# ChristophReich1996/Multi-StyleGAN

Measured on AMD Instinct MI355X. Metric: training images/sec (G+D step, 256^2, seq=3x2ch), higher is better.
Workload: dtype bf16

## Files before the change

### include/msg_hip.h

```cpp
#ifndef MSG_HIP_H
#define MSG_HIP_H

#ifdef __cplusplus
extern "C" {
#endif

enum { MSG_OK = 0, MSG_EINVAL = -1, MSG_EUNSUPPORTED = -2, MSG_ELAUNCH = -3 };
enum { MSG_F32 = 0, MSG_BF16 = 1, MSG_F16 = 2, MSG_F64 = 3, MSG_F32_SPLIT = 4 };

#define MSG_ABI_VERSION 5
int msg_abi_version(void);
const char* msg_build_arch(void);
const char* msg_strerror(int code);

int msg_upfirdn2d(const void* x, const float* fir, void* y, int dtype,
                  int major, int in_h, int in_w, int minor, int kh, int kw,
                  int up_x, int up_y, int down_x, int down_y,
                  int pad_x0, int pad_x1, int pad_y0, int pad_y1, void* stream);

int msg_upfirdn2d_pitched(const void* x, const float* fir, void* y, int dtype,
                          int major, int in_h, int in_w, int minor, int in_pitch, int kh, int kw,
                          int up_x, int up_y, int down_x, int down_y,
                          int pad_x0, int pad_x1, int pad_y0, int pad_y1, void* stream);

int msg_upfirdn2d_pitched2(const void* x, const float* fir, void* y, int dtype,
                           int major, int in_h, int in_w, int minor, int in_pitch, int out_pitch, int kh, int kw,
                           int up_x, int up_y, int down_x, int down_y,
                           int pad_x0, int pad_x1, int pad_y0, int pad_y1, void* stream);

int msg_upfirdn2d_separable(const void* x, const float* fir_y, const float* fir_x, void* y, int dtype,
                            int major, int in_h, int in_w, int minor, int kh, int kw,
                            int pad_x0, int pad_x1, int pad_y0, int pad_y1, void* stream);

int msg_upfirdn2d_separable_act(const void* x, const float* fir_y, const float* fir_x, void* y, int dtype,
                                int major, int in_h, int in_w, int minor, int kh, int kw,
                                int pad_x0, int pad_x1, int pad_y0, int pad_y1,
                                const float* act_bias, const float* noise, const float* noise_weight,
                                int noise_batch, float alpha, float scale, void* stream);
int msg_upfirdn2d_separable_act_mask(const void* x, const float* fir_y, const float* fir_x, void* y, int dtype,
                                     int major, int in_h, int in_w, int minor, int kh, int kw,
                                     int pad_x0, int pad_x1, int pad_y0, int pad_y1,
                                     const float* act_bias, const float* noise, const float* noise_weight,
                                     int noise_batch, float alpha, float scale, unsigned char* mask, void* stream);

int msg_fused_bias_act(const void* x, const float* bias, const void* ref, void* y, int dtype,
                       long long size_x, int step_b, int size_b,
                       const float* noise, const float* noise_weight, int noise_batch, int pix,
                       int act, int grad, float alpha, float scale, void* stream);

long long msg_bias_act_backward_workspace(long long size_x, int step_b, int size_b, int has_noise);
int msg_bias_act_backward(const void* gy, const void* out, void* gx, int dtype,
                          long long size_x, int step_b, int size_b,
                          float* grad_bias, const float* noise, float* grad_noise_weight,
                          int noise_batch, int pix, float alpha, float scale,
                          float* ws, long long ws_floats, void* stream);
int msg_channel_sums(const void* x, float* sums, int dtype, long long size_x, int C, float* ws, long long ws_floats,
                     void* stream);
int msg_bias_act_backward_mask(const void* gy, const unsigned char* mask, int tile_m, int tile_n, void* gx, int dtype,
                               long long size_x, int size_b,
                               float* grad_bias, const float* noise, float* grad_noise_weight,
                               int noise_batch, int pix, float alpha, float scale,
                               float* ws, long long ws_floats, void* stream);
int msg_sum_rows(const float* part, float* out, long long rows, int cols, void* stream);
int msg_bias_act_backward_mask_head(const void* gy, const void* ghead, const float* whead, const float* style,
                                    float wscale, int n_head, const unsigned char* mask, int tile_m, int tile_n,
                                    void* gx, int dtype, long long size_x, int size_b,
                                    float* grad_bias, const float* noise, float* grad_noise_weight,
                                    int noise_batch, int pix, float alpha, float scale,
                                    float* ws, long long ws_floats, void* stream);

int msg_conv2d_fprop(const void* x, const void* w, const float* bias, void* y, int dtype,
                     int B, int IH, int IW, int Cx, int Ck, int OH, int OW, int N, int ldy,
                     int kh, int kw, int stride, int pad, int in_up, int pixel_shuffle,
                     long long w_batch_stride, void* stream);
int msg_conv2d_wgrad(const void* gy, const void* x, float* gw, int dtype,
                     int B, int IH, int IW, int Cx, int I, int OH, int OW, int ldgy, int O, int ldgw,
                     int kh, int kw, int stride, int pad, int pixel_shuffle,
                     int per_sample, int k_chunks, int oi_major, float gain,
                     float* ws, long long ws_floats, void* stream);
long long msg_conv2d_wgrad_workspace(int dtype, int B, int IH, int IW, int Cx, int I, int OH, int OW, int ldgy,
                                     int O, int ldgw, int kh, int kw, int stride, int pad, int pixel_shuffle,
                                     int per_sample, int k_chunks);

int msg_demod_coeff(const float* W, const float* s, float* d, int B, int O, int I, int taps,
                    float scale, float eps, void* stream);
int msg_scale_rows_cols(const float* base, const float* rowscale, const float* colscale, void* out,
                        int dtype, int B, int R, int T, int C, int Ck, float gain, void* stream);
int msg_modulate_weights(const float* base, const float* wsq, const float* style, void* out, float* d_out,
                         int dtype, int B, int R, int O, int T, int C, int Ck, float scale, float eps, void* stream);
int msg_modulate_backward(const float* gwk, const float* W, const float* s, const float* d, float* gW,
                          float* gs_part, int B, int O, int I, int taps, int ldg, int o_group,
                          float scale, void* stream);
int msg_scale_rows_cols2(const float* base, const float* row1, const float* col1, const float* row2, const float* col2,
                         void* out, int dtype, int B, int R, int T, int C, int Ck, float gain, void* stream);
int msg_modulate_backward2(const float* gwk, const float* W, const float* s, const float* d, const float* v,
                           float* gW, float* gs_part, int B, int O, int I, int taps, int ldg, int o_group,
                           float scale, void* stream);

int msg_relayout_weight(const float* w, void* fwd, void* dgrad, float* wsq, int dtype,
                        int O, int I, int T, int Ck, int Ok, int flip, int t_major, float gain, void* stream);

int msg_gather_taps(const void* x, void* y, int dtype, int B, int H, int W, int Cx, int C, int kh, int kw,
                    int pad, int Ko, void* stream);
int msg_fold_taps(const void* g, const void* add, void* gx, int dtype, int B, int H, int W, int Ko, int C, int kh, int kw,
                  int pad, int ldx, int ld_add, void* stream);

int msg_scaled_add(const void* a, const void* b, void* y, int dtype, long long n, float beta, float gain, void* stream);
int msg_rgb_skip_merge(const void* conv, int dtype, int ld, const float* bias, const float* skip, const float* fir,
                       float* out, int B, int C, int H, int W, void* stream);
int msg_rgb_skip_merge_backward(const float* g, void* g_conv, int dtype, int ld, float* g_skip, const float* fir,
                                int B, int C, int H, int W, void* stream);
int msg_gamma_merge(const void* a, const void* b, const float* gamma, void* y, int dtype, long long n, float gain, void* stream);
long long msg_gamma_merge_backward_workspace(void);
int msg_gamma_merge_backward(const void* gy, const void* a, const float* gamma, void* ga, void* gb, float* g_gamma, int dtype,
                             long long n, float gain, float* ws, void* stream);
int msg_scaled_add_rows(const void* a, const void* b, void* y, int dtype, long long rows, int cols,
                        long long lda, long long ldb, long long ldy, float beta, float gain, void* stream);

int msg_softmax_rows(const void* x, void* y, int dtype, long long rows, int cols, void* stream);
int msg_softmax_rows_backward(const void* y, const void* gy, void* gx, int dtype, long long rows, int cols,
                              void* stream);
int msg_softmax_rows_backward2(const void* y, const void* gy, const void* v, void* d_y, void* d_gy, int dtype,
                               long long rows, int cols, void* stream);

int msg_nonlocal_attention_supported(int B, int Nq, int Nk, int dk, int dv);
int msg_nonlocal_attention_fwd(const void* q, const void* k, const void* vt, void* o, float* lse, int dtype,
                               int B, int Nq, int Nk, int dk, int dv, void* stream);
int msg_maxpool2x2_fwd(const void* x, void* y, unsigned short* idx, int dtype, int B, int H, int W, int C, long long ldx,
                       void* stream);
int msg_maxpool2x2_bwd(const void* gy, const unsigned short* idx, void* gx, int dtype, int B, int H, int W, int C,
                       void* stream);
int msg_maxpool2x2_gather(const void* v, const unsigned short* idx, void* out, int dtype, int B, int H, int W, int C,
                          long long ldv, void* stream);

int msg_nonlocal_attention_bwd_splits(int B, int Nq, int Nk);
int msg_nonlocal_attention_bwd(const void* q, const void* qt, const void* k, const void* kt, const void* v,
                               const void* dO, const void* dOt, const void* o, const float* lse, float* delta,
                               void* dq, void* dk_out, void* dv_out, float* workspace, int dtype,
                               int B, int Nq, int Nk, int dk, int dv, void* stream);

int msg_affine_warp(const float* x, float* y, const float* angle_deg, float angle_const, const float* scale_xy,
                    const float* select_u, const float* p, int rot_prob, float cx, float cy, int padding,
                    int align_corners, int B, int C, int H, int W, int backward, void* workspace, void* stream);

long long msg_minibatch_stddev_workspace(int C, int H, int W, int groups, int dtype);
int msg_minibatch_stddev(const void* x, void* y, float* stat, float* workspace, int dtype,
                         int B, int C, int H, int W, int ldx, int ldy, int groups, float alpha, void* stream);
int msg_minibatch_stddev_backward(const void* x, const void* gy, const float* gstat, void* gx, int dtype,
                                  int B, int C, int H, int W, int ldx, int ldgy, int ldgx, int groups,
                                  float alpha, void* stream);

int msg_conv2d_fprop_act(const void* x, const void* w, void* y, int dtype,
                         int B, int IH, int IW, int Cx, int Ck, int OH, int OW, int N, int ldy,
                         int kh, int kw, int stride, int pad, long long w_batch_stride,
                         const float* act_bias, const float* noise, const float* noise_weight,
                         int noise_batch, float alpha, float scale, void* stream);
int msg_conv2d_fprop_act_mask(const void* x, const void* w, void* y, int dtype,
                              int B, int IH, int IW, int Cx, int Ck, int OH, int OW, int N, int ldy,
                              int kh, int kw, int stride, int pad, long long w_batch_stride,
                              const float* act_bias, const float* noise, const float* noise_weight,
                              int noise_batch, float alpha, float scale, unsigned char* mask, void* stream);

int msg_conv2d_fprop_residual(const void* x, const void* w, void* y, int dtype,
                              int B, int IH, int IW, int Cx, int Ck, int OH, int OW, int N, int ldy,
                              int kh, int kw, int stride, int pad, long long w_batch_stride,
                              const void* residual, int res_ld, float gain, void* stream);

long long msg_conv2d_fprop_act_backward_workspace(int dtype, int B, int IH, int IW, int Cx, int Ck, int OH, int OW,
                                                  int N, int kh, int kw, long long w_batch_stride, int has_noise);
int msg_conv2d_fprop_act_backward(const void* x, const void* w, void* y, int dtype,
                                  int B, int IH, int IW, int Cx, int Ck, int OH, int OW, int N, int ldy,
                                  int kh, int kw, int stride, int pad, long long w_batch_stride,
                                  const void* residual, int res_ld,
                                  const unsigned char* sign_mask, int mask_tile_m, int mask_tile_n,
                                  const void* sign_map, int sign_ld, float alpha, float scale,
// ... 50 lines not shown
```

### multi_stylegan_amd/conv_ops.py

```python
import math
import os
from typing import Optional, Tuple

import torch
from torch.autograd import Function

from . import _lib
from ._autograd import _derive


def _vec(dtype) -> int:
    return 8 if dtype == torch.bfloat16 else 4


def _round_up(n: int, m: int) -> int:
    return (n + m - 1) // m * m


def _padded_nhwc(b, c, h, w, dtype, device):
    cx = _round_up(c, _vec(dtype))
    buf = torch.empty((b, h, w, cx), dtype=dtype, device=device)
    if cx != c:
        buf[..., c:].zero_()
    return buf.permute(0, 3, 1, 2)[:, :c]
# ... 1498 lines not shown


class _ModConvGrad(Function):

    @staticmethod
    def forward(ctx, gy, x, weight, style, d, demodulate, upsample, g, scale, need):
        gx, gw, gs, gwk = _modconv_backward(x, weight, style, d, gy, demodulate, upsample, g, scale, need, keep_gwk=True)
        ctx.set_materialize_grads(False)
        ctx.save_for_backward(gy, x, weight, style, d, gwk)
        ctx.cfg = (demodulate, upsample, g, scale)
        return gx, gw, gs

    @staticmethod
    @torch.autograd.function.once_differentiable
    def backward(ctx, a, cot_w, cot_s):
        gy, x, weight, style, d, gwk = ctx.saved_tensors
        demodulate, upsample, g, scale = ctx.cfg
        want = ctx.needs_input_grad[:4]
        _, o, i, kh, kw = weight.shape
        b, t = x.shape[0], kh * kw
        tail = (None,) * 6
        if a is None and cot_w is None and cot_s is None:
            return (None, None, None, None) + tail
        if cot_w is not None or i % 4 or i > 512 or t not in (1, 4, 9) or b > _MODCONV_BWD_BATCH or \
                (cot_s is not None and gwk is None):
            return _modconv_second_order_composite(gy, x, weight, style, demodulate, upsample, a, cot_w, cot_s, want) + tail
        dev = x.device
        w3 = weight.detach().reshape(o, i, t)
        s = style.detach().float().contiguous()
        dd = d if demodulate else None
        esz = 2 if gy.dtype == torch.bfloat16 else 4
        ck, okp = _round_up(i, 128 // esz), _round_up(o, 128 // esz)
        rows = t * o if upsample else o
        ggy = gx2 = gw3 = gs2 = None
        if a is not None:
            a = a.to(x.dtype)
            if want[0]:
                wk = torch.empty((b, rows, 1 if upsample else t, ck), dtype=x.dtype, device=dev)
                base = _fwd_image_base(weight, w3, upsample, g.kind)
                if demodulate:
                    _scale_rows_cols(base, d.repeat(1, t) if upsample else d, s, wk, scale)
                else:
                    _scale_rows_cols(base, None, s, wk, scale)
                ggy = _fprop_modconv(a, wk, ck, o, i, kh, kw, upsample, g)
            if want[2] or want[3]:
                gwk_a, ldg = _wgrad_modconv(gy, a, o, i, kh, kw, upsample, g)
                gw3, gs2 = _fold_weight_gradient(gwk_a, ldg, w3, s, dd, scale, style.dtype)
        if cot_s is not None:
            v = cot_s.detach().float().contiguous()
            if want[0] or want[1]:
                hf = torch.empty((b, rows, 1 if upsample else t, ck), dtype=x.dtype, device=dev)
                hd = torch.empty((b, i, t, okp), dtype=gy.dtype, device=dev)
                base_f = _fwd_image_base(weight, w3, upsample, g.kind)
                base_d = _dgrad_image_base(weight, w3, upsample, g.kind)
                if demodulate:
                    wsq = _tap_square_sums(weight, w3, g.kind)
                    ddir = -(scale * scale) * d.pow(3) * linear(s * v, wsq)
                    rows_d, rows_dd = (d.repeat(1, t), ddir.repeat(1, t)) if upsample else (d, ddir)
                    with _lib.on_device(dev):
                        lib, st = _lib.lib(), _lib.stream_of(dev)
                        code = lib.msg_scale_rows_cols2(base_f.data_ptr(), rows_d.contiguous().data_ptr(), v.data_ptr(),
                                                        rows_dd.contiguous().data_ptr(), s.data_ptr(), hf.data_ptr(),
                                                        _lib.dtype_code(hf), b, rows, 1 if upsample else t, i, ck, scale, st)
                        _lib.check(code, "msg_scale_rows_cols2")
                        code = lib.msg_scale_rows_cols2(base_d.data_ptr(), v.data_ptr(), d.data_ptr(), s.data_ptr(),
                                                        ddir.contiguous().data_ptr(), hd.data_ptr(), _lib.dtype_code(hd), b, i, t,
                                                        o, okp, scale, st)
                        _lib.check(code, "msg_scale_rows_cols2")
                else:
                    _scale_rows_cols(base_f, None, v, hf, scale)
                    _scale_rows_cols(base_d, v, None, hd, scale)
                if want[0]:
                    ggy = _fprop_modconv(x, hf, ck, o, i, kh, kw, upsample, g, add_to=ggy)
                if want[1]:
                    gx2 = _dgrad_modconv(gy, hd, okp, o, i, kh, kw, upsample, g)
            if want[2] or want[3]:
                gw3b, gs2b = _fold_weight_gradient(gwk, gwk.shape[-1], w3, s, dd, scale, style.dtype, cotangent=v)
                gw3 = gw3b if gw3 is None else gw3 + gw3b
                gs2 = gs2b if gs2 is None else gs2 + gs2b
        gw = gw3.reshape(1, o, i, kh, kw) if (gw3 is not None and want[2]) else None
        return (ggy, gx2, gw, gs2 if want[3] else None) + tail


class _ModulatedConv(Function):

    @staticmethod
    def forward(ctx, x, weight, style, demodulate, upsample, act_bias=None, noise=None, noise_w=None, alpha=0.2,
                act_scale=1.0, fuse_act=False, head_slot=None, input_act=None):
        dev = _lib.require_gpu(x, weight, style)
        ctx.input_act = input_act if input_act is not None and input_act.armed else None
        ctx.head_slot = head_slot
        if head_slot is not None and fuse_act:
            ctx.set_materialize_grads(False)
            head_slot.armed = True
        _, o, i, kh, kw = weight.shape
        b, t = x.shape[0], kh * kw
        scale = math.sqrt(2.0) / math.sqrt(i * t)
        w3 = weight.detach().reshape(o, i, t)
        s = style.detach().float().contiguous()
        d = None
        esz = 2 if x.dtype == torch.bfloat16 else 4
        ck = _round_up(i, 128 // esz)
        kind = "up2" if upsample else "conv"
        img = _param_images(weight, torch.float32, 1.0, kind, modulation=True)
        base = img["f"][0] if img is not None else _cached(weight, "mb" + kind, torch.float32, 1.0, lambda: (
            (w3.permute(2, 0, 1).reshape(t * o, 1, i) if upsample else w3.transpose(1, 2)).contiguous(), 0))[0]
        rows = t * o if upsample else o
        wk = torch.empty((b, rows, 1 if upsample else t, ck), dtype=x.dtype, device=dev)
        if demodulate:
            wsq = img["wsq"] if img is not None else \
                _cached(weight, "wsq", torch.float32, 1.0, lambda: (w3.square().sum(dim=2).contiguous(), 0))[0]
            d = torch.empty((b, o), dtype=torch.float32, device=dev)
            with _lib.on_device(dev):
                code = _lib.lib().msg_modulate_weights(base.data_ptr(), wsq.data_ptr(), s.data_ptr(), wk.data_ptr(),
                                                       d.data_ptr(), _lib.dtype_code(wk), b, rows, o,
                                                       1 if upsample else t, i, ck, scale, 1e-8, _lib.stream_of(dev))
            _lib.check(code, "msg_modulate_weights")
        else:
            _scale_rows_cols(base, None, s, wk, scale)
        g = Geometry(kind, kh, kw, 1, kh // 2, x.shape[2:], True)
        act = None
        holder = [] if any(ctx.needs_input_grad) else None
        if fuse_act:
            assert not upsample, "the upsampling layers blur before their activation"
            act = (*_act_operands(act_bias, noise, noise_w, (b, o, *g.y_hw)), alpha, act_scale, holder)
        if upsample:
            y = _launch_fprop(x, wk, ck, None, 4 * o, g.x_hw, 1, 1, 1, 0, 1, True, True, i, mode=g.mode)
        else:
            y = _launch_fprop(x, wk, ck, None, o, g.y_hw, kh, kw, 1, kh // 2, 1, False, True, i, act=act, mode=g.mode)
        ctx.save_for_backward(x, weight, style, d if d is not None else torch.empty(0, device=dev),
                              y if fuse_act else None, noise if fuse_act else None)
        ctx.cfg = (demodulate, upsample, g, scale)
        ctx.act = (alpha, act_scale, act_bias is not None, noise is not None,
                   None if noise_w is None else noise_w.shape) if fuse_act else None
        ctx.bias_param = act_bias
        ctx.mask = holder[0] if holder else None
        return y

    @staticmethod
    def backward(ctx, gy):
        x, weight, style, d, y_act, noise = ctx.saved_tensors
        demodulate, upsample, g, scale = ctx.cfg
        _, o, i, kh, kw = weight.shape
        b, t = x.shape[0], kh * kw
        need = list(ctx.needs_input_grad)
        need[1], need[2] = _consumed(ctx, 1, 1), _consumed(ctx, 2, 2)
        gb = gnw = None
        slot = ctx.head_slot
        if ctx.act is not None:
            from .op_static.fused_act import FusedLeakyReLUFunctionBackward, act_backward_with_head
            alpha, act_scale, has_bias, has_noise, nw_shape = ctx.act
            head, head_dgrad = slot.take() if slot is not None else (None, None)
            fused = None
            if head is not None:
                fused = act_backward_with_head(gy, head, y_act.shape, noise if has_noise else None,
                                               ctx.bias_param if has_bias else None, has_bias, alpha, act_scale, ctx.mask)
                if fused is None:
                    gh = head_dgrad()
                    gy = gh if gy is None else gy + gh
            if fused is not None:
                gy, gb, gnw = fused
            elif gy is None:
                return (None,) * 13
            else:
                gy, gb, gnw = _derive(FusedLeakyReLUFunctionBackward, gy, y_act, noise if has_noise else None,
                                      ctx.bias_param if has_bias else False, alpha, act_scale, ctx.mask)
            gb = gb if has_bias and need[5] else None
            gnw = gnw.reshape(nw_shape) if has_noise and need[7] else None
        tail = (None, None, gb, None, gnw, None, None, None, None, None)
        if ctx.act is None and slot is not None and slot.armed and need[0] and not torch.is_grad_enabled() and \
                fused_head_ok(gy, weight, b, demodulate, upsample):
            gyc, wt, st = gy, weight, style
            slot.head = (gyc, weight.detach().reshape(o, i).float().contiguous(), style.detach().float().contiguous(), scale)
            slot.dgrad = lambda: _modconv_backward(x, wt, st, d, gyc, demodulate, upsample, g, scale,
                                                   [True, False, False])[0]
            need[0] = False
        fused_ok = i <= 512 and t <= 9
        if torch.is_grad_enabled() and fused_ok and _NATIVE_SECOND_ORDER and b <= _MODCONV_BWD_BATCH and x.is_cuda:
            gx, gw, gs = _derive(_ModConvGrad, gy, x, weight, style, d if demodulate else None, demodulate, upsample, g, scale,
                                            tuple(need[:3]))
            return (gx, gw, gs) + tail
        if torch.is_grad_enabled() or not fused_ok:
            with torch.enable_grad():
                ins = [v for v, n in zip((x, weight, style), need[:3]) if n]
                y2 = _modulated_composite(x, weight, style, demodulate, upsample)
                grads = list(torch.autograd.grad(y2, ins, gy, create_graph=torch.is_grad_enabled(), allow_unused=True))
            out = [grads.pop(0) if n else None for n in need[:3]]
            return (out[0], out[1], out[2]) + tail
        if b > _MODCONV_BWD_BATCH:
            gxs, gws, gss = [], [], []
            for lo in range(0, b, _MODCONV_BWD_BATCH):
                hi = min(b, lo + _MODCONV_BWD_BATCH)
                cgx, cgw, cgs = _modconv_backward(x[lo:hi], weight, style[lo:hi], d[lo:hi] if demodulate else d,
                                                  gy[lo:hi], demodulate, upsample, g, scale, need)
                gxs.append(cgx); gws.append(cgw); gss.append(cgs)
            gx = torch.cat(gxs) if need[0] else None
            gw = torch.stack(gws).sum(dim=0) if gws[0] is not None else None
            gs = torch.cat(gss) if gss[0] is not None else None
            return (gx, gw, gs) + tail
        gx, gw, gs = _modconv_backward(x, weight, style, d, gy, demodulate, upsample, g, scale, need, direct=True,
                                       act_bwd=ctx.input_act)
        return (gx, gw, gs) + tail


def fused_head_ok(gy, weight, b, demodulate, upsample) -> bool:
    _, o, _, kh, kw = weight.shape
    return gy is not None and gy.is_cuda and gy.dtype == torch.bfloat16 and kh == 1 and kw == 1 and o <= 8 and \
        not demodulate and not upsample and b <= _MODCONV_BWD_BATCH and HEAD_GRAD_FUSION

# ... 16 lines not shown
```

### multi_stylegan_amd/csrc/modulate.hip

```cpp
#include "msg_common.h"
#include <stdlib.h>

__device__ __forceinline__ float block_sum_256(float v, float* red ) {
    v = wave_sum(v);
    __syncthreads();
    if ((threadIdx.x & 63) == 0) red[threadIdx.x >> 6] = v;
    __syncthreads();
    return red[0] + red[1] + red[2] + red[3];
}

__global__ __launch_bounds__(256) void demod_coeff_kernel(const float* __restrict__ W, const float* __restrict__ s,
                                                          float* __restrict__ d, int B, int O, int I, int T,
                                                          float scale, float eps) {
    __shared__ float red[4];
    const int o = blockIdx.x;
    const float* wo = W + (size_t)o * I * T;
    for (int b = 0; b < B; ++b) {
        float acc = 0.f;
        for (int i = threadIdx.x; i < I; i += 256) {
            const float sv = s[(size_t)b * I + i];
            float w2 = 0.f;
            for (int t = 0; t < T; ++t) { const float wv = wo[i * T + t]; w2 = fmaf(wv, wv, w2); }
            acc = fmaf(w2, sv * sv, acc);
        }
// ... 96 lines not shown
        hipLaunchKernelGGL((scale_rows_cols_kernel<bf16_t>), grid, dim3(256), 0, s, base, rowscale, colscale,
                           (bf16_t*)out, B, bg, R, T, C, Ck, gain);
    else
        hipLaunchKernelGGL((scale_rows_cols_kernel<float>), grid, dim3(256), 0, s, base, rowscale, colscale,
                           (float*)out, B, bg, R, T, C, Ck, gain);
    return MSG_CHECK_LAUNCH();
}

template <typename TO>
__global__ __launch_bounds__(256) void scale_rows_cols2_kernel(const float* __restrict__ base,
                                                               const float* __restrict__ row1, const float* __restrict__ col1,
                                                               const float* __restrict__ row2, const float* __restrict__ col2,
                                                               TO* __restrict__ out, int B, int BG, int R, int T, int C, int Ck,
                                                               float gain) {
    using V = Vec16<TO>;
    constexpr int VEC = V::N;
    const int r = blockIdx.x, b0 = blockIdx.y * BG, b1 = min(B, b0 + BG);
    const int cvecs = Ck / VEC;
    const float* src_row = base + (size_t)r * T * C;
    const int tstep = 256 / cvecs > 0 ? 256 / cvecs : 1;
    const bool al = (C % 4 == 0) && ((((uintptr_t)base | (uintptr_t)col1 | (uintptr_t)col2) & 15u) == 0);
    for (int cv = threadIdx.x % cvecs; cv < cvecs; cv += 256) {
        const int c0 = cv * VEC;
        const int t0 = threadIdx.x / cvecs;
        for (int tb = t0; tb < T; tb += tstep * SRC_ITEMS) {
            float f[SRC_ITEMS][VEC];
#pragma unroll
            for (int k = 0; k < SRC_ITEMS; ++k) {
                const int t = tb + k * tstep;
                if (t < T) load_run<VEC>(src_row + (size_t)t * C, c0, C, al, f[k]);
                else {
#pragma unroll
                    for (int e = 0; e < VEC; ++e) f[k][e] = 0.f;
                }
            }
            for (int b = b0; b < b1; ++b) {
                const float rs1 = gain * row1[(size_t)b * R + r], rs2 = gain * row2[(size_t)b * R + r];
                float sc[VEC], s2[VEC];
                load_run<VEC>(col1 + (size_t)b * C, c0, C, al, sc);
                load_run<VEC>(col2 + (size_t)b * C, c0, C, al, s2);
#pragma unroll
                for (int e = 0; e < VEC; ++e) sc[e] = fmaf(rs1, sc[e], rs2 * s2[e]);
                TO* dst_row = out + ((size_t)b * R + r) * T * Ck;
#pragma unroll
                for (int k = 0; k < SRC_ITEMS; ++k) {
                    const int t = tb + k * tstep;
                    if (t >= T) break;
                    V o;
                    if constexpr (VEC == 4) {
#pragma unroll
                        for (int e = 0; e < 4; ++e) o.set(e, f[k][e] * sc[e]);
                    } else {
#pragma unroll
                        for (int e = 0; e < 4; ++e) o.set2(e, f[k][2 * e] * sc[2 * e], f[k][2 * e + 1] * sc[2 * e + 1]);
                    }
                    *reinterpret_cast<uint4*>(dst_row + (size_t)t * Ck + c0) = o.raw;
                }
            }
        }
    }
}

extern "C" int msg_scale_rows_cols2(const float* base, const float* row1, const float* col1, const float* row2,
                                    const float* col2, void* out, int dtype, int B, int R, int T, int C, int Ck, float gain,
                                    void* stream) {
    if (B == 0) return MSG_OK;
    if (!base || !row1 || !col1 || !row2 || !col2 || !out || B < 0 || R <= 0 || T <= 0 || C <= 0 || Ck < C) return MSG_EINVAL;
    if (dtype != MSG_F32 && dtype != MSG_BF16) return MSG_EUNSUPPORTED;
    const int vec = dtype == MSG_BF16 ? 8 : 4;
    if (Ck % vec || (((uintptr_t)out) & 15u)) return MSG_EUNSUPPORTED;
    hipStream_t s = (hipStream_t)stream;
    int bg = 1;
    while (bg < 8 && bg * 2 <= B && (long long)R * ((B + 2 * bg - 1) / (2 * bg)) >= 2048) bg *= 2;
    dim3 grid(R, (B + bg - 1) / bg);
    if (dtype == MSG_BF16)
        hipLaunchKernelGGL((scale_rows_cols2_kernel<bf16_t>), grid, dim3(256), 0, s, base, row1, col1, row2, col2,
                           (bf16_t*)out, B, bg, R, T, C, Ck, gain);
    else
        hipLaunchKernelGGL((scale_rows_cols2_kernel<float>), grid, dim3(256), 0, s, base, row1, col1, row2, col2,
                           (float*)out, B, bg, R, T, C, Ck, gain);
    return MSG_CHECK_LAUNCH();
}

template <typename TO>
__global__ __launch_bounds__(256) void modulate_weights_kernel(const float* __restrict__ base, const float* __restrict__ wsq,
                                                               const float* __restrict__ style, TO* __restrict__ out,
                                                               float* __restrict__ d_out, int B, int BG, int R, int O,
                                                               int T, int C, int Ck, float scale, float eps) {
    using V = Vec16<TO>;
    constexpr int VEC = V::N;
    __shared__ float red[4 * 8];
    __shared__ float dsh[8];
    const int o = blockIdx.x, b0 = blockIdx.y * BG, b1 = min(B, b0 + BG);
    {
        float part[8];
#pragma unroll
        for (int k = 0; k < 8; ++k) part[k] = 0.f;
        for (int i = threadIdx.x; i < C; i += 256) {
            const float q = wsq[(size_t)o * C + i];
#pragma unroll
            for (int k = 0; k < 8; ++k)
                if (b0 + k < b1) { const float sv = style[(size_t)(b0 + k) * C + i]; part[k] = fmaf(q, sv * sv, part[k]); }
        }
#pragma unroll
        for (int k = 0; k < 8; ++k) {
            const float v = wave_sum(part[k]);
            if ((threadIdx.x & 63) == 0) red[(threadIdx.x >> 6) * 8 + k] = v;
        }
        __syncthreads();
        if (threadIdx.x < 8 && b0 + (int)threadIdx.x < b1) {
            const int k = threadIdx.x;
            const float tot = red[k] + red[8 + k] + red[16 + k] + red[24 + k];
            const float dv = rsqrtf(scale * scale * tot + eps);
            dsh[k] = dv;
            if (d_out) d_out[(size_t)(b0 + k) * O + o] = dv;
        }
        __syncthreads();
    }
    const int cvecs = Ck / VEC;
    const int tstep = 256 / cvecs > 0 ? 256 / cvecs : 1;
    const bool al = (C % 4 == 0) && ((((uintptr_t)base | (uintptr_t)style) & 15u) == 0);
    const int npairs = (R / O) * T;
    for (int cv = threadIdx.x % cvecs; cv < cvecs; cv += 256) {
        const int c0 = cv * VEC;
        const int t0 = threadIdx.x / cvecs;
        for (int qb = t0; qb < npairs; qb += tstep * SRC_ITEMS) {
            float f[SRC_ITEMS][VEC];
            size_t cell[SRC_ITEMS];
#pragma unroll
            for (int k = 0; k < SRC_ITEMS; ++k) {
                const int q = qb + k * tstep;
                const int rk = q / T, t = q - rk * T;
                cell[k] = (size_t)(o + rk * O) * T + t;
                if (q < npairs) load_run<VEC>(base + cell[k] * C, c0, C, al, f[k]);
                else {
#pragma unroll
                    for (int e = 0; e < VEC; ++e) f[k][e] = 0.f;
                }
            }
            for (int b = b0; b < b1; ++b) {
                const float rs = scale * dsh[b - b0];
                float sc[VEC];
                load_run<VEC>(style + (size_t)b * C, c0, C, al, sc);
#pragma unroll
                for (int e = 0; e < VEC; ++e) sc[e] *= rs;
                TO* dst_b = out + (size_t)b * R * T * Ck;
#pragma unroll
                for (int k = 0; k < SRC_ITEMS; ++k) {
                    if (qb + k * tstep >= npairs) break;
                    V ov;
                    if constexpr (VEC == 4) {
#pragma unroll
                        for (int e = 0; e < 4; ++e) ov.set(e, f[k][e] * sc[e]);
                    } else {
#pragma unroll
                        for (int e = 0; e < 4; ++e) ov.set2(e, f[k][2 * e] * sc[2 * e], f[k][2 * e + 1] * sc[2 * e + 1]);
                    }
                    *reinterpret_cast<uint4*>(dst_b + cell[k] * Ck + c0) = ov.raw;
                }
            }
        }
    }
}

extern "C" int msg_modulate_weights(const float* base, const float* wsq, const float* style, void* out, float* d_out,
                                    int dtype, int B, int R, int O, int T, int C, int Ck, float scale, float eps,
                                    void* stream) {
    if (B == 0) return MSG_OK;
    if (!base || !wsq || !style || !out || B < 0 || R <= 0 || O <= 0 || R % O || T <= 0 || C <= 0 || Ck < C) return MSG_EINVAL;
    if (dtype != MSG_F32 && dtype != MSG_BF16) return MSG_EUNSUPPORTED;
    const int vec = dtype == MSG_BF16 ? 8 : 4;
    if (Ck % vec || ((uintptr_t)out & 15u) || B > 65535) return MSG_EUNSUPPORTED;
    hipStream_t s = (hipStream_t)stream;
    static const int min_wgs = msg_tunable("MSG_MODW_MIN_WGS", 1024);
    int bg = 1;
    while (bg < 8 && bg * 2 <= B && (long long)O * ((B + 2 * bg - 1) / (2 * bg)) >= min_wgs) bg *= 2;
    dim3 grid(O, (B + bg - 1) / bg);
    if (dtype == MSG_BF16)
        hipLaunchKernelGGL((modulate_weights_kernel<bf16_t>), grid, dim3(256), 0, s, base, wsq, style, (bf16_t*)out, d_out,
                           B, bg, R, O, T, C, Ck, scale, eps);
    else
        hipLaunchKernelGGL((modulate_weights_kernel<float>), grid, dim3(256), 0, s, base, wsq, style, (float*)out, d_out,
                           B, bg, R, O, T, C, Ck, scale, eps);
    return MSG_CHECK_LAUNCH();
}

constexpr int MB_SLOTS = 2;
constexpr int MB_TAPS = 9;
constexpr int MB_BMAX = 32;
template <bool DEMOD>
__global__ __launch_bounds__(256) void modulate_backward_kernel(const float* __restrict__ gwk, const float* __restrict__ W,
                                                                const float* __restrict__ s, const float* __restrict__ d,
                                                                float* __restrict__ gW, float* __restrict__ gs_part,
                                                                int B, int O, int I, int T, int ldg, int OG, float scale) {
    __shared__ float red[4 * MB_BMAX];
    __shared__ float Tsh[MB_BMAX];
    const int og = blockIdx.x;
    const int tid = threadIdx.x, lane = tid & 63, wid = tid >> 6;
    float gs_acc[MB_BMAX / 2][MB_SLOTS];
#pragma unroll
    for (int b = 0; b < MB_BMAX / 2; ++b)
// ... 418 lines not shown
```

Measured before the change: 156.5.

## Add fused small-resolution modulated conv that modulates weights in-register

For low-resolution layers (up to 64 pixels for 3x3, 16 for the 2x2 upsample path), a new kernel applies style modulation and demodulation to the fp32 base weights in registers and feeds them straight into bf16 MFMA. This avoids materialising per-sample modulated weight tensors. The K dimension is split across slices and summed by a second kernel that also applies the bias/noise/leaky-ReLU epilogue and the pixel shuffle. Demod coefficients now come from a separate small kernel. The cost is a partial-sum workspace, an extra reduce launch, and recomputing the weight modulation in every block.

```diff
diff --git a/include/msg_hip.h b/include/msg_hip.h
--- a/include/msg_hip.h
+++ b/include/msg_hip.h
@@ -91,6 +91,18 @@
 int msg_modulate_backward(const float* gwk, const float* W, const float* s, const float* d, float* gW,
                           float* gs_part, int B, int O, int I, int taps, int ldg, int o_group,
                           float scale, void* stream);
+int msg_demod_coefficients(const float* wsq, const float* style, float* d_out, int B, int O, int C, float scale, float eps,
+                           void* stream);
+long long msg_modconv_small_workspace(int B, int H, int W, int C, int N, int kh, int pixel_shuffle);
+int msg_modconv_small_fprop(const void* x, const float* base, const float* style, const float* d, void* y, int B,
+                            int H, int W, int Cx, int C, int N, int O, int ldy, int kh, int pixel_shuffle,
+                            float scale, const float* act_bias, const float* noise, const float* noise_weight,
+                            int noise_batch, int act, float alpha, float act_scale, unsigned char* mask, float* ws,
+                            long long ws_floats, void* stream);
+long long msg_modconv_small_probe_workspace(int B, int H, int W, int C, int N, int kh);
+int msg_modconv_small_probe(const void* x, const float* base, const float* style, const float* d, void* y, int B,
+                            int H, int W, int Cx, int C, int N, int O, int ldy, int kh, int pixel_shuffle,
+                            float scale, float* ws, long long ws_floats, void* stream);
 int msg_scale_rows_cols2(const float* base, const float* row1, const float* col1, const float* row2, const float* col2,
                          void* out, int dtype, int B, int R, int T, int C, int Ck, float gain, void* stream);
 int msg_modulate_backward2(const float* gwk, const float* W, const float* s, const float* d, const float* v,
diff --git a/multi_stylegan_amd/conv_ops.py b/multi_stylegan_amd/conv_ops.py
--- a/multi_stylegan_amd/conv_ops.py
+++ b/multi_stylegan_amd/conv_ops.py
@@ -1604,6 +1604,48 @@
         return (ggy, gx2, gw, gs2 if want[3] else None) + tail
 
 
+MODCONV_SMALL = bool(int(os.environ.get("MSG_MODCONV_SMALL", "1")))
+_MODSMALL_WS: dict = {}
+modconv_small_launches = [0]
+
+
+def _modconv_small_workspace(x, b, i, rows, kh, kw, upsample) -> int:
+    if not MODCONV_SMALL or x.dtype != torch.bfloat16 or not x.is_cuda or b == 0 or \
+            (kh, kw) != ((2, 2) if upsample else (3, 3)):
+        return 0
+    key = (b, x.shape[2], x.shape[3], i, rows, upsample)
+    ws = _MODSMALL_WS.get(key)
+    if ws is None:
+        ws = _MODSMALL_WS[key] = max(0, _lib.lib().msg_modconv_small_workspace(b, x.shape[2], x.shape[3], i, rows,
+                                                                              1 if upsample else 3, int(upsample)))
+    return ws
+
+
+def _launch_modconv_small(x, base, s, d, o, i, upsample, scale, act, ws_floats, mask=None):
+    dev = _lib.require_gpu(x, base, s, d)
+    xv, cx = _nhwc_view(x)
+    b, _, h, w = xv.shape
+    n = 4 * o if upsample else o
+    y, ldy = _alloc_out(b, o, 2 * h, 2 * w, x.dtype, dev) if upsample else _alloc_out(b, o, h, w, x.dtype, dev)
+    act_bias = noise = noise_w = None
+    alpha = act_scale = 0.0
+    if act is not None:
+        act_bias, noise, noise_w, alpha, act_scale = act[:5]
+        _lib.require_gpu(x, act_bias, noise, noise_w)
+    key = "modconv_small"
+    if _lib.kernel_clock.enabled and _CLOCK_SHAPES:
+        key += f"|B{b} {h}x{w} {i}->{n} {'up' if upsample else '3x3'}|"
+    modconv_small_launches[0] += 1
+    with _lib.on_device(dev), _lib.kernel_clock.span((key, 'bf16'), 2.0 * b * h * w * n * (1 if upsample else 9) * i):
+        code = _lib.lib().msg_modconv_small_fprop(
+            xv.data_ptr(), base.data_ptr(), s.data_ptr(), _lib.ptr(d), y.data_ptr(), b, h, w, cx, i, n, o, ldy,
+            1 if upsample else 3, int(upsample), float(scale), _lib.ptr(act_bias), _lib.ptr(noise), _lib.ptr(noise_w),
+            1 if noise is None else noise.shape[0], int(act is not None), float(alpha), float(act_scale), _lib.ptr(mask),
+            _lib.scratch_ptr(ws_floats, dev), ws_floats, _lib.stream_of(dev))
+    _lib.check(code, "msg_modconv_small_fprop")
+    return y
+
+
 class _ModulatedConv(Function):
 
     @staticmethod
@@ -1628,8 +1670,18 @@
         base = img["f"][0] if img is not None else _cached(weight, "mb" + kind, torch.float32, 1.0, lambda: (
             (w3.permute(2, 0, 1).reshape(t * o, 1, i) if upsample else w3.transpose(1, 2)).contiguous(), 0))[0]
         rows = t * o if upsample else o
-        wk = torch.empty((b, rows, 1 if upsample else t, ck), dtype=x.dtype, device=dev)
-        if demodulate:
+        small_ws = _modconv_small_workspace(x, b, i, rows, kh, kw, upsample)
+        wk = None if small_ws else torch.empty((b, rows, 1 if upsample else t, ck), dtype=x.dtype, device=dev)
+        if small_ws:
+            if demodulate:
+                wsq = img["wsq"] if img is not None else \
+                    _cached(weight, "wsq", torch.float32, 1.0, lambda: (w3.square().sum(dim=2).contiguous(), 0))[0]
+                d = torch.empty((b, o), dtype=torch.float32, device=dev)
+                with _lib.on_device(dev):
+                    code = _lib.lib().msg_demod_coefficients(wsq.data_ptr(), s.data_ptr(), d.data_ptr(), b, o, i, scale, 1e-8,
+                                                             _lib.stream_of(dev))
+                _lib.check(code, "msg_demod_coefficients")
+        elif demodulate:
             wsq = img["wsq"] if img is not None else \
                 _cached(weight, "wsq", torch.float32, 1.0, lambda: (w3.square().sum(dim=2).contiguous(), 0))[0]
             d = torch.empty((b, o), dtype=torch.float32, device=dev)
@@ -1646,7 +1698,9 @@
         if fuse_act:
             assert not upsample, "the upsampling layers blur before their activation"
             act = (*_act_operands(act_bias, noise, noise_w, (b, o, *g.y_hw)), alpha, act_scale, holder)
-        if upsample:
+        if small_ws:
+            y = _launch_modconv_small(x, base, s, d, o, i, upsample, scale, act, small_ws)
+        elif upsample:
             y = _launch_fprop(x, wk, ck, None, 4 * o, g.x_hw, 1, 1, 1, 0, 1, True, True, i, mode=g.mode)
         else:
             y = _launch_fprop(x, wk, ck, None, o, g.y_hw, kh, kw, 1, kh // 2, 1, False, True, i, act=act, mode=g.mode)
diff --git a/multi_stylegan_amd/csrc/conv_modsmall.hip b/multi_stylegan_amd/csrc/conv_modsmall.hip
--- /dev/null
+++ b/multi_stylegan_amd/csrc/conv_modsmall.hip
@@ -0,0 +1,285 @@
+#include "msg_common.h"
+
+typedef __bf16 bf16v8 __attribute__((ext_vector_type(8)));
+
+constexpr int MODSMALL_MAX_PIX_3X3 = 64;
+constexpr int MODSMALL_MAX_PIX_UP = 16;
+constexpr int MODSMALL_HARD_MAX_PIX = 256;
+
+struct ModSmallArgs {
+    const bf16_t* x;
+    const float* base;
+    const float* style;
+    const float* d;
+    float* part;
+    int B, H, W, Cx, C, N, O, taps, P, KT, Lr;
+    float scale;
+};
+
+struct ModSmallPlan {
+    int ok, mb, z, ksteps, slices, lr, kt;
+};
+
+static ModSmallPlan modsmall_plan(int B, int H, int W, int C, int N, int taps, int max_pix) {
+    ModSmallPlan p = {0, 0, 0, 0, 0, 0, 0};
+    const long long P = (long long)H * W;
+    if (B <= 0 || H <= 0 || W <= 0 || (taps != 1 && taps != 9) || C <= 0 || N <= 0 || C % 64 || N % 64) return p;
+    if (P > max_pix || P % 16 || B > 65535) return p;
+    const int blocks = (int)P / 16;
+    int z = blocks >= 16 ? 4 : blocks >= 2 ? 2 : 1;
+    if (blocks % z || (blocks / z != 1 && blocks / z != 2 && blocks / z != 4)) z = blocks;
+    p.z = z;
+    p.mb = blocks / z;
+    p.kt = taps * (C / 32);
+    const int opts[4] = {9, 4, 2, 1};
+    int slices = (p.kt + 3) / 4;
+    for (int k = 0; k < 4; ++k) {
+        const int s = (p.kt + 4 * opts[k] - 1) / (4 * opts[k]);
+        if ((long long)(N / 32) * z * s >= 256 || k == 3) { slices = s; break; }
+    }
+    p.slices = slices;
+    p.lr = (p.kt + slices - 1) / slices;
+    const int need = (p.lr + 3) / 4;
+    p.ksteps = need <= 1 ? 1 : need <= 2 ? 2 : need <= 4 ? 4 : 9;
+    p.ok = need <= 9;
+    return p;
+}
+
+template <int MB, int KSTEPS>
+__global__ __launch_bounds__(256) void modsmall_contract_kernel(const ModSmallArgs a) {
+    __shared__ float4 red[2][4][2 * MB][64];
+    const int lane = threadIdx.x & 63, w = threadIdx.x >> 6;
+    const int n0 = blockIdx.x * 32, slice = blockIdx.y, blk0 = blockIdx.z * MB;
+    const int lr = lane & 15, cslot = (lane >> 4) * 8;
+    const int cpt = a.C >> 5;
+    const int ks0 = slice * a.Lr, ks1 = min(ks0 + a.Lr, a.KT);
+
+    float fb[KSTEPS][2][8];
+    int soff[KSTEPS];
+    int xoff[KSTEPS][MB];
+#pragma unroll
+    for (int i = 0; i < KSTEPS; ++i) {
+        const int ks = ks0 + w + 4 * i;
+        const bool ok = ks < ks1;
+        const int tap = ok ? ks / cpt : 0;
+        const int c = (ok ? (ks - tap * cpt) * 32 : 0) + cslot;
+        soff[i] = ok ? c : -1;
+#pragma unroll
+        for (int nt = 0; nt < 2; ++nt) {
+            const float* src = a.base + ((size_t)(n0 + nt * 16 + lr) * a.taps + tap) * a.C + c;
+            const f32x4 lo = ok ? *reinterpret_cast<const f32x4*>(src) : f32x4{0.f, 0.f, 0.f, 0.f};
+            const f32x4 hi = ok ? *reinterpret_cast<const f32x4*>(src + 4) : f32x4{0.f, 0.f, 0.f, 0.f};
+#pragma unroll
+            for (int e = 0; e < 4; ++e) { fb[i][nt][e] = lo[e]; fb[i][nt][4 + e] = hi[e]; }
+        }
+        const int dy = a.taps == 9 ? tap / 3 - 1 : 0, dx = a.taps == 9 ? tap - (tap / 3) * 3 - 1 : 0;
+#pragma unroll
+        for (int mb = 0; mb < MB; ++mb) {
+            const int pix = (blk0 + mb) * 16 + lr;
+            const int oh = pix / a.W, ow = pix - oh * a.W;
+            const int ih = oh + dy, iw = ow + dx;
+            const bool in = ok && ih >= 0 && ih < a.H && iw >= 0 && iw < a.W;
+            xoff[i][mb] = in ? (ih * a.W + iw) * a.Cx + c : -1;
+        }
+    }
+    const int orow[2] = {(n0 + lr) % a.O, (n0 + 16 + lr) % a.O};
+    const size_t xs = (size_t)a.P * a.Cx;
+
+    u32x4 xb[KSTEPS][MB];
+    f32x4 sv[KSTEPS][2];
+    float dv[2];
+    auto fetch = [&](int b) {
+        const bf16_t* xp = a.x + (size_t)b * xs;
+        const float* sp = a.style + (size_t)b * a.C;
+#pragma unroll
+        for (int i = 0; i < KSTEPS; ++i) {
+            const bool ok = soff[i] >= 0;
+            sv[i][0] = ok ? *reinterpret_cast<const f32x4*>(sp + soff[i]) : f32x4{0.f, 0.f, 0.f, 0.f};
+            sv[i][1] = ok ? *reinterpret_cast<const f32x4*>(sp + soff[i] + 4) : f32x4{0.f, 0.f, 0.f, 0.f};
+#pragma unroll
+            for (int mb = 0; mb < MB; ++mb)
+                xb[i][mb] = xoff[i][mb] >= 0 ? *reinterpret_cast<const u32x4*>(xp + xoff[i][mb]) : u32x4{0u, 0u, 0u, 0u};
+        }
+#pragma unroll
+        for (int nt = 0; nt < 2; ++nt) dv[nt] = a.d ? a.d[(size_t)b * a.O + orow[nt]] : 1.f;
+    };
+
+    constexpr bool PREFETCH = KSTEPS < 9;
+    if constexpr (PREFETCH) fetch(0);
+    for (int b = 0; b < a.B; ++b) {
+        if constexpr (!PREFETCH) fetch(b);
+        u32x4 xc[KSTEPS][MB];
+        f32x4 sc4[KSTEPS][2];
+        float rs[2];
+#pragma unroll
+        for (int i = 0; i < KSTEPS; ++i) {
+            sc4[i][0] = sv[i][0]; sc4[i][1] = sv[i][1];
+#pragma unroll
+            for (int mb = 0; mb < MB; ++mb) xc[i][mb] = xb[i][mb];
+        }
+        rs[0] = a.scale * dv[0]; rs[1] = a.scale * dv[1];
+        if constexpr (PREFETCH) { if (b + 1 < a.B) fetch(b + 1); }
+
+        f32x4 acc[2][MB];
+#pragma unroll
+        for (int nt = 0; nt < 2; ++nt)
+#pragma unroll
+            for (int mb = 0; mb < MB; ++mb) acc[nt][mb] = f32x4{0.f, 0.f, 0.f, 0.f};
+#pragma unroll
+        for (int i = 0; i < KSTEPS; ++i) {
+            if (soff[i] < 0) continue;
+#pragma unroll
+            for (int nt = 0; nt < 2; ++nt) {
+                float sc[8];
+#pragma unroll
+                for (int e = 0; e < 4; ++e) { sc[e] = sc4[i][0][e] * rs[nt]; sc[4 + e] = sc4[i][1][e] * rs[nt]; }
+                u32x4 wp;
+#pragma unroll
+                for (int e = 0; e < 4; ++e)
+                    wp[e] = (uint32_t)f2bf(fb[i][nt][2 * e] * sc[2 * e]) | ((uint32_t)f2bf(fb[i][nt][2 * e + 1] * sc[2 * e + 1]) << 16);
+                const bf16v8 wf = __builtin_bit_cast(bf16v8, wp);
+#pragma unroll
+                for (int mb = 0; mb < MB; ++mb)
+                    acc[nt][mb] = __builtin_amdgcn_mfma_f32_16x16x32_bf16(wf, __builtin_bit_cast(bf16v8, xc[i][mb]), acc[nt][mb], 0, 0, 0);
+            }
+        }
+        const int buf = b & 1;
+#pragma unroll
+        for (int nt = 0; nt < 2; ++nt)
+#pragma unroll
+            for (int mb = 0; mb < MB; ++mb) {
+                const f32x4 v = acc[nt][mb];
+                red[buf][w][nt * MB + mb][lane] = make_float4(v[0], v[1], v[2], v[3]);
+            }
+        __syncthreads();
+        for (int u = w; u < 2 * MB; u += 4) {
+            float4 s = red[buf][0][u][lane];
+#pragma unroll
+            for (int k = 1; k < 4; ++k) {
+                const float4 t = red[buf][k][u][lane];
+                s.x += t.x; s.y += t.y; s.z += t.z; s.w += t.w;
+            }
+            const int nt = u / MB, mb = u - nt * MB;
+            const int pix = (blk0 + mb) * 16 + lr;
+            const int n = n0 + nt * 16 + (lane >> 4) * 4;
+            *reinterpret_cast<float4*>(a.part + (((size_t)slice * a.B + b) * a.P + pix) * a.N + n) = s;
+        }
+    }
+}
+
+struct ModSmallEpi {
+    const float* part;
+    bf16_t* y;
+    int B, H, W, N, ldy, slices, pixel_shuffle;
+    ActEpilogue act;
+};
+
+__global__ __launch_bounds__(256) void modsmall_reduce_kernel(const ModSmallEpi e) {
+    const int nv8 = e.N >> 3, P = e.H * e.W;
+    const long long idx = (long long)blockIdx.x * 256 + threadIdx.x;
+    if (idx >= (long long)e.B * P * nv8) return;
+    const long long q = idx / nv8;
+    const int cv = (int)(idx - q * nv8), n = cv * 8;
+    const int b = (int)(q / P), pix = (int)(q - (long long)b * P);
+    const float* p = e.part + (size_t)q * e.N + n;
+    const size_t stride = (size_t)e.B * P * e.N;
+    f32x4 lo = *reinterpret_cast<const f32x4*>(p), hi = *reinterpret_cast<const f32x4*>(p + 4);
+    for (int s = 1; s < e.slices; ++s) {
+        lo += *reinterpret_cast<const f32x4*>(p + s * stride);
+        hi += *reinterpret_cast<const f32x4*>(p + s * stride + 4);
+    }
+    u32x4 v;
+    v[0] = (uint32_t)f2bf(lo[0]) | ((uint32_t)f2bf(lo[1]) << 16);
+    v[1] = (uint32_t)f2bf(lo[2]) | ((uint32_t)f2bf(lo[3]) << 16);
+    v[2] = (uint32_t)f2bf(hi[0]) | ((uint32_t)f2bf(hi[1]) << 16);
+    v[3] = (uint32_t)f2bf(hi[2]) | ((uint32_t)f2bf(hi[3]) << 16);
+    if (e.act.enabled == 1) {
+        float bv[8];
+#pragma unroll
+        for (int k = 0; k < 8; ++k) bv[k] = e.act.bias ? e.act.bias[n + k] : 0.f;
+        const float nw = e.act.noise ? e.act.noise_w[0] : 0.f;
+        const float nv = e.act.noise ? nw * e.act.noise[(long long)(e.act.noise_batch == 1 ? 0 : b) * P + pix] : 0.f;
+        v = act_epilogue_apply<bf16_t>(v, bv, nv, e.act.alpha, e.act.scale);
+        if (e.act.mask) e.act.mask[q * nv8 + cv] = (unsigned char)act_sign_byte(v);
+    }
+    long long g = q;
+    int nn = n;
+    if (e.pixel_shuffle) {
+        const int oc = e.N >> 2, qd = n / oc;
+        nn = n - qd * oc;
+        const int oh = pix / e.W, ow = pix - oh * e.W;
+        g = ((long long)b * 2 * e.H + 2 * oh + (qd >> 1)) * (2 * e.W) + 2 * ow + (qd & 1);
+    }
+    *reinterpret_cast<u32x4*>(e.y + g * e.ldy + nn) = v;
+}
+
+extern "C" long long msg_modconv_small_workspace(int B, int H, int W, int C, int N, int kh, int pixel_shuffle) {
+    if (B == 0) return 0;
+    if ((kh != 1 && kh != 3) || (kh == 3) == (pixel_shuffle != 0)) return MSG_EUNSUPPORTED;
+    const ModSmallPlan p = modsmall_plan(B, H, W, C, N, kh * kh, pixel_shuffle ? MODSMALL_MAX_PIX_UP : MODSMALL_MAX_PIX_3X3);
+    return p.ok ? (long long)p.slices * B * H * W * N : (long long)MSG_EUNSUPPORTED;
+}
+
+template <int MB>
+static bool modsmall_launch(const ModSmallPlan& p, const ModSmallArgs& a, hipStream_t st) {
+    const dim3 grid(a.N / 32, p.slices, p.z);
+    switch (p.ksteps) {
+        case 1: hipLaunchKernelGGL((modsmall_contract_kernel<MB, 1>), grid, dim3(256), 0, st, a); return true;
+        case 2: hipLaunchKernelGGL((modsmall_contract_kernel<MB, 2>), grid, dim3(256), 0, st, a); return true;
+        case 4: hipLaunchKernelGGL((modsmall_contract_kernel<MB, 4>), grid, dim3(256), 0, st, a); return true;
+        case 9: hipLaunchKernelGGL((modsmall_contract_kernel<MB, 9>), grid, dim3(256), 0, st, a); return true;
+        default: return false;
+    }
+}
+
+static int modsmall_fprop(const void* x, const float* base, const float* style, const float* d, void* y, int B, int H, int W,
+                          int Cx, int C, int N, int O, int ldy, int kh, int pixel_shuffle, float scale, const float* act_bias,
+                          const float* noise, const float* noise_weight, int noise_batch, int act, float alpha, float act_scale,
+                          unsigned char* mask, float* ws, long long ws_floats, int max_pix, void* stream) {
+    if (B == 0) return MSG_OK;
+    if (!x || !base || !style || !y || !ws || B < 0 || O <= 0 || (act != 0 && act != 1)) return MSG_EINVAL;
+    if ((kh != 1 && kh != 3) || (kh == 3) == (pixel_shuffle != 0)) return MSG_EUNSUPPORTED;
+    if (N != (pixel_shuffle ? 4 * O : O) || (act && pixel_shuffle) || (mask && !act)) return MSG_EUNSUPPORTED;
+    if (act && noise && (!noise_weight || (noise_batch != 1 && noise_batch != B))) return MSG_EINVAL;
+    const ModSmallPlan p = modsmall_plan(B, H, W, C, N, kh * kh, max_pix);
+    if (!p.ok || O % 64) return MSG_EUNSUPPORTED;
+    if (Cx < C || Cx % 8 || ldy % 8 || ldy < (pixel_shuffle ? O : N)) return MSG_EUNSUPPORTED;
+    if ((((uintptr_t)x | (uintptr_t)base | (uintptr_t)style | (uintptr_t)y | (uintptr_t)ws) & 15u)) return MSG_EUNSUPPORTED;
+    if ((long long)H * W * Cx * (long long)B >= (1ll << 31)) return MSG_EUNSUPPORTED;
+    if (ws_floats < (long long)p.slices * B * H * W * N) return MSG_EINVAL;
+    hipStream_t st = (hipStream_t)stream;
+    ModSmallArgs a{(const bf16_t*)x, base, style, d, ws, B, H, W, Cx, C, N, O, kh * kh, H * W, p.kt, p.lr, scale};
+    const bool ok = p.mb == 1 ? modsmall_launch<1>(p, a, st) : p.mb == 2 ? modsmall_launch<2>(p, a, st)
+                  : p.mb == 4 ? modsmall_launch<4>(p, a, st) : false;
+    if (!ok) return MSG_EUNSUPPORTED;
+    ModSmallEpi e{};
+    e.part = ws; e.y = (bf16_t*)y;
+    e.B = B; e.H = H; e.W = W; e.N = N; e.ldy = ldy; e.slices = p.slices; e.pixel_shuffle = pixel_shuffle;
+    e.act.enabled = act;
+    e.act.bias = act_bias; e.act.noise = noise; e.act.noise_w = noise_weight; e.act.noise_batch = noise_batch;
+    e.act.alpha = alpha; e.act.scale = act_scale; e.act.mask = mask;
+    const long long threads = (long long)B * H * W * (N / 8);
+    hipLaunchKernelGGL(modsmall_reduce_kernel, dim3((unsigned)((threads + 255) / 256)), dim3(256), 0, st, e);
+    return MSG_CHECK_LAUNCH();
+}
+
+extern "C" int msg_modconv_small_fprop(const void* x, const float* base, const float* style, const float* d, void* y, int B,
+                                       int H, int W, int Cx, int C, int N, int O, int ldy, int kh, int pixel_shuffle,
+                                       float scale, const float* act_bias, const float* noise, const float* noise_weight,
+                                       int noise_batch, int act, float alpha, float act_scale, unsigned char* mask, float* ws,
+                                       long long ws_floats, void* stream) {
+    return modsmall_fprop(x, base, style, d, y, B, H, W, Cx, C, N, O, ldy, kh, pixel_shuffle, scale, act_bias, noise,
+                          noise_weight, noise_batch, act, alpha, act_scale, mask, ws, ws_floats,
+                          pixel_shuffle ? MODSMALL_MAX_PIX_UP : MODSMALL_MAX_PIX_3X3, stream);
+}
+
+extern "C" long long msg_modconv_small_probe_workspace(int B, int H, int W, int C, int N, int kh) {
+    const ModSmallPlan p = modsmall_plan(B, H, W, C, N, kh * kh, MODSMALL_HARD_MAX_PIX);
+    return p.ok ? (long long)p.slices * B * H * W * N : (long long)MSG_EUNSUPPORTED;
+}
+extern "C" int msg_modconv_small_probe(const void* x, const float* base, const float* style, const float* d, void* y, int B,
+                                       int H, int W, int Cx, int C, int N, int O, int ldy, int kh, int pixel_shuffle,
+                                       float scale, float* ws, long long ws_floats, void* stream) {
+    return modsmall_fprop(x, base, style, d, y, B, H, W, Cx, C, N, O, ldy, kh, pixel_shuffle, scale, nullptr, nullptr, nullptr,
+                          1, 0, 0.f, 1.f, nullptr, ws, ws_floats, MODSMALL_HARD_MAX_PIX, stream);
+}
diff --git a/multi_stylegan_amd/csrc/modulate.hip b/multi_stylegan_amd/csrc/modulate.hip
--- a/multi_stylegan_amd/csrc/modulate.hip
+++ b/multi_stylegan_amd/csrc/modulate.hip
@@ -202,6 +202,53 @@
     return MSG_CHECK_LAUNCH();
 }
 
+__device__ __forceinline__ void demod_row_coefficients(const float* __restrict__ wsq, const float* __restrict__ style,
+                                                       float* __restrict__ d_out, int o, int b0, int b1, int O, int C,
+                                                       float scale, float eps, float* red , float* dsh ) {
+    float part[8];
+#pragma unroll
+    for (int k = 0; k < 8; ++k) part[k] = 0.f;
+    for (int i = threadIdx.x; i < C; i += 256) {
+        const float q = wsq[(size_t)o * C + i];
+#pragma unroll
+        for (int k = 0; k < 8; ++k)
+            if (b0 + k < b1) { const float sv = style[(size_t)(b0 + k) * C + i]; part[k] = fmaf(q, sv * sv, part[k]); }
+    }
+#pragma unroll
+    for (int k = 0; k < 8; ++k) {
+        const float v = wave_sum(part[k]);
+        if ((threadIdx.x & 63) == 0) red[(threadIdx.x >> 6) * 8 + k] = v;
+    }
+    __syncthreads();
+    if (threadIdx.x < 8 && b0 + (int)threadIdx.x < b1) {
+        const int k = threadIdx.x;
+        const float tot = red[k] + red[8 + k] + red[16 + k] + red[24 + k];
+        const float dv = rsqrtf(scale * scale * tot + eps);
+        dsh[k] = dv;
+        if (d_out) d_out[(size_t)(b0 + k) * O + o] = dv;
+    }
+    __syncthreads();
+}
+
+__global__ __launch_bounds__(256) void demod_coefficients_kernel(const float* __restrict__ wsq, const float* __restrict__ style,
+                                                                 float* __restrict__ d_out, int B, int O, int C, float scale,
+                                                                 float eps) {
+    __shared__ float red[4 * 8];
+    __shared__ float dsh[8];
+    const int b0 = blockIdx.y * 8;
+    demod_row_coefficients(wsq, style, d_out, blockIdx.x, b0, min(B, b0 + 8), O, C, scale, eps, red, dsh);
+}
+
+extern "C" int msg_demod_coefficients(const float* wsq, const float* style, float* d_out, int B, int O, int C, float scale,
+                                      float eps, void* stream) {
+    if (B == 0) return MSG_OK;
+    if (!wsq || !style || !d_out || B < 0 || O <= 0 || C <= 0) return MSG_EINVAL;
+    if ((B + 7) / 8 > 65535) return MSG_EUNSUPPORTED;
+    hipLaunchKernelGGL(demod_coefficients_kernel, dim3(O, (B + 7) / 8), dim3(256), 0, (hipStream_t)stream, wsq, style, d_out, B,
+                       O, C, scale, eps);
+    return MSG_CHECK_LAUNCH();
+}
+
 template <typename TO>
 __global__ __launch_bounds__(256) void modulate_weights_kernel(const float* __restrict__ base, const float* __restrict__ wsq,
                                                                const float* __restrict__ style, TO* __restrict__ out,
@@ -212,31 +259,7 @@
     __shared__ float red[4 * 8];
     __shared__ float dsh[8];
     const int o = blockIdx.x, b0 = blockIdx.y * BG, b1 = min(B, b0 + BG);
-    {
-        float part[8];
-#pragma unroll
-        for (int k = 0; k < 8; ++k) part[k] = 0.f;
-        for (int i = threadIdx.x; i < C; i += 256) {
-            const float q = wsq[(size_t)o * C + i];
-#pragma unroll
-            for (int k = 0; k < 8; ++k)
-                if (b0 + k < b1) { const float sv = style[(size_t)(b0 + k) * C + i]; part[k] = fmaf(q, sv * sv, part[k]); }
-        }
-#pragma unroll
-        for (int k = 0; k < 8; ++k) {
-            const float v = wave_sum(part[k]);
-            if ((threadIdx.x & 63) == 0) red[(threadIdx.x >> 6) * 8 + k] = v;
-        }
-        __syncthreads();
-        if (threadIdx.x < 8 && b0 + (int)threadIdx.x < b1) {
-            const int k = threadIdx.x;
-            const float tot = red[k] + red[8 + k] + red[16 + k] + red[24 + k];
-            const float dv = rsqrtf(scale * scale * tot + eps);
-            dsh[k] = dv;
-            if (d_out) d_out[(size_t)(b0 + k) * O + o] = dv;
-        }
-        __syncthreads();
-    }
+    demod_row_coefficients(wsq, style, d_out, o, b0, b1, O, C, scale, eps, red, dsh);
     const int cvecs = Ck / VEC;
     const int tstep = 256 / cvecs > 0 ? 256 / cvecs : 1;
     const bool al = (C % 4 == 0) && ((((uintptr_t)base | (uintptr_t)style) & 15u) == 0);
```

After: 155.4. About the same (-0.7%).
